# claserken/SISS

Hardware: AMD Instinct MI355X
Metric: unlearning samples/sec (= unlearning-steps/sec x batch x gpus), CelebA-HQ-256 DDPM SISS (higher is better)
Workload: dtype bf16; 1 GPU; delete_celeb.yaml: CelebA-HQ 256x256 DDPM UNet (113.7M params), SISS lambd=0.5, t=999, bf16, bs=16/GPU, GA=1, scaling_norm=500, AdamW lr 5e-6; loss_fn=importance_sampling_with_mixture, global_batch=16, grad_accum=1, parallelism=dp1, hipgraph=True

## Files before the change

### siss_amd/csrc/groupnorm.hip

```cpp
#include "nt_common.h"

namespace {

constexpr int kStatsDepth = 2;
constexpr int kThreads = 256;
constexpr int kMaxG = 32;
constexpr int kMaxC = 1024;

struct GNShape {
    int H, W, C, G, cpg, lpp, ppi;
    int chunk_px, nchunks;
    int ld, Gf, nslices;
    int ldx;
};

__device__ __forceinline__ long compact_row(int n, int pi, int H, int W) { return (long)n * H * W + pi; }

__device__ __forceinline__ void unpack8(u32x4_t r, float (&v)[8]) {
#pragma unroll
    for (int j = 0; j < 4; ++j) {
        v[2 * j] = __builtin_bit_cast(float, r[j] << 16);
        v[2 * j + 1] = __builtin_bit_cast(float, r[j] & 0xffff0000u);
    }
}
__device__ __forceinline__ u32x4_t pack8(const float (&v)[8]) {
    return u32x4_t{pack_bf2(v[0], v[1]), pack_bf2(v[2], v[3]), pack_bf2(v[4], v[5]), pack_bf2(v[6], v[7])};
}

struct PixelWalk {
    int pi, p1, x, W, ppi, dx, rw, drw;
    __device__ __forceinline__ PixelWalk(const GNShape& s, int chunk, int slot) {
        const int p0 = chunk * s.chunk_px;
        p1 = p0 + s.chunk_px; p1 = p1 < s.H * s.W ? p1 : s.H * s.W;
        pi = p0 + slot; W = s.W; ppi = s.ppi;
        const int y = pi / W; x = pi - y * W;
        const int dy = ppi / W; dx = ppi - dy * W;
        rw = (y + 1) * (W + 2) + (x + 1);
        drw = dy * (W + 2) + dx;
    }
    __device__ __forceinline__ bool ok() const { return pi < p1; }
    __device__ __forceinline__ int row() const { return rw; }
    __device__ __forceinline__ void next() {
        pi += ppi; x += dx; rw += drw;
        if (x >= W) { x -= W; rw += 2; }
    }
};

__device__ __forceinline__ unsigned boff(int row, unsigned row_bytes, unsigned lane_bytes) { return __umul24(row, row_bytes) + lane_bytes; }
__device__ __forceinline__ u32x4_t ld16(const bf16_t* base, unsigned off) {
    return *reinterpret_cast<const u32x4_t*>(reinterpret_cast<const char*>(base) + off);
}
__device__ __forceinline__ void st16(bf16_t* base, unsigned off, u32x4_t v) {
    *reinterpret_cast<u32x4_t*>(reinterpret_cast<char*>(base) + off) = v;
}

__device__ __forceinline__ void reduce_slots(const float (&v)[8], bool active, int slot, int cc, const GNShape& s,
                                             float* red, float* out) {
    if (active) {
        float* dst = red + slot * s.C + cc * 8;
        *reinterpret_cast<f32x4_t*>(dst) = f32x4_t{v[0], v[1], v[2], v[3]};
        *reinterpret_cast<f32x4_t*>(dst + 4) = f32x4_t{v[4], v[5], v[6], v[7]};
    }
    __syncthreads();
    for (int c = threadIdx.x; c < s.C; c += kThreads) {
        float a = 0.f;
        for (int sl = 0; sl < s.ppi; ++sl) a += red[sl * s.C + c];
        out[c] = a;
    }
    __syncthreads();
}

__global__ __launch_bounds__(kThreads) void gn_stats_kernel(const bf16_t* __restrict__ x, GNShape s,
                                                            float* __restrict__ partial) {
    __shared__ __attribute__((aligned(16))) float red[2048];
    __shared__ float ch_a[kMaxC], ch_b[kMaxC];
    const int n = blockIdx.y, chunk = blockIdx.x, tid = threadIdx.x;
    const int c0 = blockIdx.z * s.C;
    const int slot = tid / s.lpp, cc = tid - slot * s.lpp;
    const bool active = slot < s.ppi;
    float a[8] = {}, b[8] = {};
    if (active) {
        const bf16_t* base = x + (long)n * (s.H + 2) * (s.W + 2) * s.ldx + c0;
        const unsigned xb = s.ldx * 2, lb = cc * 16;
        PixelWalk w(s, chunk, slot);
        while (w.ok()) {
            const u32x4_t r0 = ld16(base, boff(w.row(), xb, lb));
            w.next();
// ... 106 lines not shown

__global__ __launch_bounds__(kThreads) void gn_qstats_finalize_kernel(
    const float* __restrict__ qsA, int qa, const float* __restrict__ qsB, int qb, int H, int W, int G, int cpg, float eps,
    float* __restrict__ mean, float* __restrict__ rstd) {
    const int n = blockIdx.x, tid = threadIdx.x, lane = tid & 63;
    const int g = blockIdx.y * 4 + (tid >> 6);
    if (g >= G) return;
    const long rpi = (long)(H + 2) * (W + 2);
    const int t0 = (int)(n * rpi / kQsTileRows), t1 = (int)(((n + 1) * rpi - 1) / kQsTileRows);
    const int qpg = cpg >> 2;
    const int items = (t1 - t0 + 1) * 2 * qpg;
    auto entry = [&](int it) -> float2 {
        if (it >= items) return float2{0.f, 0.f};
        const int hl = it / qpg, qi = it - hl * qpg;
        const int t = t0 + (hl >> 1), h = hl & 1;
        const int slot = (int)((long)t * kQsTileRows / rpi) == n ? 0 : 1;
        const int q = g * qpg + qi;
        const float* src = q < qa ? qsA : qsB;
        const int stride = q < qa ? qa : qb, qq = q < qa ? q : q - qa;
        return *reinterpret_cast<const float2*>(src + (((long)(2 * t + h) * 2 + slot) * stride + qq) * 2);
    };
    double a = 0.0, b = 0.0;
    for (int it = lane; it < items; it += 256) {
        const float2 e0 = entry(it), e1 = entry(it + 64), e2 = entry(it + 128), e3 = entry(it + 192);
        a += ((double)e0.x + (double)e1.x) + ((double)e2.x + (double)e3.x);
        b += ((double)e0.y + (double)e1.y) + ((double)e2.y + (double)e3.y);
    }
#pragma unroll
    for (int o = 32; o >= 1; o >>= 1) { a += __shfl_xor(a, o); b += __shfl_xor(b, o); }
    if (lane == 0) {
        const double cnt = (double)H * W * cpg;
        const double m = a / cnt;
        double var = b / cnt - m * m;
        var = var > 0 ? var : 0;
        mean[(long)n * G + g] = (float)m;
        rstd[(long)n * G + g] = (float)(1.0 / sqrt(var + (double)eps));
    }
}

__global__ __launch_bounds__(kThreads) void gn_quad_stats_kernel(const bf16_t* __restrict__ x, long ld, int M, int N, int rpi,
                                                                 float* __restrict__ qs) {
    __shared__ float red[8][kThreads];
    const int t = blockIdx.x >> 1, h = blockIdx.x & 1, tid = threadIdx.x;
    const int r0 = t * kQsTileRows + h * kQsHalfRows;
    int r1 = r0 + (h ? kQsTileRows - kQsHalfRows : kQsHalfRows);
    r1 = r1 < M ? r1 : M;
    const int bnd = (t * kQsTileRows / rpi + 1) * rpi;
    const int lpr = N >> 3, par = kThreads / lpr;
    const int rr = tid / lpr, cc = tid - rr * lpr;
    float a[8];
#pragma unroll
    for (int i = 0; i < 8; ++i) a[i] = 0.f;
    if (rr < par) {
        const bf16_t* src = x + cc * 8;
        for (int r = r0 + rr; r < r1; r += par) {
            const u32x4_t v4 = *reinterpret_cast<const u32x4_t*>(src + (long)r * ld);
            float v[8];
            unpack8(v4, v);
            const float w1 = r >= bnd ? 1.f : 0.f, w0 = 1.f - w1;
#pragma unroll
            for (int j = 0; j < 2; ++j) {
                const float s1 = (v[4 * j] + v[4 * j + 1]) + (v[4 * j + 2] + v[4 * j + 3]);
                const float s2 = (v[4 * j] * v[4 * j] + v[4 * j + 1] * v[4 * j + 1]) + (v[4 * j + 2] * v[4 * j + 2] + v[4 * j + 3] * v[4 * j + 3]);
                a[4 * j] += w0 * s1; a[4 * j + 1] += w0 * s2;
                a[4 * j + 2] += w1 * s1; a[4 * j + 3] += w1 * s2;
            }
        }
    }
#pragma unroll
    for (int i = 0; i < 8; ++i) red[i][tid] = a[i];
    __syncthreads();
    if (tid < lpr * 4) {
        const int c = tid >> 2, j = (tid >> 1) & 1, slot = tid & 1;
        float s1 = 0.f, s2 = 0.f;
        for (int k = 0; k < par; ++k) {
            s1 += red[4 * j + 2 * slot][k * lpr + c];
            s2 += red[4 * j + 2 * slot + 1][k * lpr + c];
        }
        const long e = ((long)(2 * t + h) * 2 + slot) * (N >> 2) + (2 * c + j);
        *reinterpret_cast<float2*>(qs + 2 * e) = float2{s1, s2};
    }
}

template <bool SILU, int SETS>
__global__ __launch_bounds__(kThreads) void gn_bwd_stats_kernel(
    const bf16_t* __restrict__ dy, const bf16_t* __restrict__ x, const float* __restrict__ gamma,
    const float* __restrict__ beta, const float* __restrict__ mean, const float* __restrict__ rstd,
    GNShape s, int nx, int dy_compact, int set_images, long set_stride, float* __restrict__ partial,
    float* __restrict__ dgamma, float* __restrict__ dbeta) {
    __shared__ __attribute__((aligned(16))) float red[2048];
    __shared__ float ch1[kMaxC], ch2[kMaxC];
    const int n = blockIdx.y, chunk = blockIdx.x, tid = threadIdx.x;
    const int c0 = blockIdx.z * s.C, g0 = blockIdx.z * s.G;
    const int slot = tid / s.lpp, cc = tid - slot * s.lpp;
    const bool active = slot < s.ppi;
    gamma += c0; beta += c0; dy += c0;
    float a1[SETS][8], a2[SETS][8];
#pragma unroll
    for (int k = 0; k < SETS; ++k)
#pragma unroll
        for (int e = 0; e < 8; ++e) { a1[k][e] = 0.f; a2[k][e] = 0.f; }
    if (active) {
        float mr[8], rs[8], ga[8], be[8], ga2[8], be2[8];
#pragma unroll
        for (int e = 0; e < 8; ++e) {
            const int c = cc * 8 + e, g = c / s.cpg;
            rs[e] = rstd[(long)n * s.Gf + g0 + g]; mr[e] = mean[(long)n * s.Gf + g0 + g] * rs[e];
            ga[e] = gamma[c]; be[e] = beta[c];
            ga2[e] = -1.44269504088896f * ga[e]; be2[e] = -1.44269504088896f * be[e];
        }
        const long rpi = (long)(s.H + 2) * (s.W + 2);
        const bf16_t* xbase = x + (long)n * rpi * s.ldx + c0;
        const bf16_t* dbase[SETS];
#pragma unroll
        for (int k = 0; k < SETS; ++k)
            dbase[k] = dy + (dy_compact ? (long)(k * nx + n) * s.H * s.W : (long)(k * nx + n) * rpi) * s.ld;
        const unsigned xb = s.ldx * 2, db = s.ld * 2, lb = cc * 16;
        PixelWalk w(s, chunk, slot);
        constexpr int DEPTH = kStatsDepth;
        u32x4_t bx[DEPTH], bd[DEPTH][SETS];
        bool have[DEPTH];
        auto issue = [&](const PixelWalk& q, u32x4_t& ox, u32x4_t (&od)[SETS]) {
            ox = ld16(xbase, boff(q.row(), xb, lb));
            const unsigned doff = boff(dy_compact ? q.pi : q.row(), db, lb);
#pragma unroll
            for (int k = 0; k < SETS; ++k) od[k] = ld16(dbase[k], doff);
        };
#pragma unroll
        for (int b2 = 0; b2 < DEPTH; ++b2) {
            bx[b2] = u32x4_t{0u, 0u, 0u, 0u};
#pragma unroll
            for (int k = 0; k < SETS; ++k) bd[b2][k] = u32x4_t{0u, 0u, 0u, 0u};
            have[b2] = w.ok();
            if (have[b2]) { issue(w, bx[b2], bd[b2]); w.next(); }
        }
        while (have[0]) {
#pragma unroll
            for (int b2 = 0; b2 < DEPTH; ++b2) {
                if (!have[b2]) break;
                const u32x4_t rx = bx[b2];
                u32x4_t rd[SETS];
#pragma unroll
                for (int k = 0; k < SETS; ++k) rd[k] = bd[b2][k];
                have[b2] = w.ok();
                if (have[b2]) { issue(w, bx[b2], bd[b2]); w.next(); }
                float v[8], q1[8], q2[8];
                unpack8(rx, v);
#pragma unroll
                for (int e = 0; e < 8; ++e) {
                    const float xh = v[e] * rs[e] - mr[e];
                    if (SILU) {
                        const float ex = __builtin_amdgcn_exp2f(xh * ga2[e] + be2[e]);
                        const float sg = __builtin_amdgcn_rcpf(1.f + ex);
                        const float z = xh * ga[e] + be[e];
                        q1[e] = sg * (1.f + z * (1.f - sg));
                    } else {
                        q1[e] = 1.f;
                    }
                    q2[e] = q1[e] * xh;
                }
#pragma unroll
                for (int k = 0; k < SETS; ++k) {
                    float d[8];
                    unpack8(rd[k], d);
#pragma unroll
                    for (int e = 0; e < 8; ++e) {
                        a1[k][e] += d[e] * q1[e]; a2[k][e] += d[e] * q2[e];
                    }
                }
            }
        }
    }
    for (int k = 0; k < SETS; ++k) {
        reduce_slots(a1[k], active, slot, cc, s, red, ch1);
        reduce_slots(a2[k], active, slot, cc, s, red, ch2);
        const int n2 = k * nx + n;
        if (tid < 2 * s.G) {
            const int g = tid >> 1;
            const float* src = (tid & 1) ? ch2 : ch1;
            float t = 0.f;
            for (int c = g * s.cpg; c < (g + 1) * s.cpg; ++c) t += src[c] * gamma[c];
            partial[(((long)n2 * s.nslices + blockIdx.z) * s.nchunks + chunk) * 2 * s.G + tid] = t;
        }
        const long so = (long)(n2 / set_images) * set_stride + c0;
        for (int i = tid; i < s.C; i += kThreads) {
            atomicAdd(dgamma + so + i, ch2[i]);
            atomicAdd(dbeta + so + i, ch1[i]);
        }
        __syncthreads();
    }
}

template <bool SILU>
__device__ __forceinline__ void gn_bwd_xhat(float v, float rs, float mr, float ga, float be, float& xh, float& dsl) {
#pragma clang fp contract(off)
    xh = fmaf(v, rs, -mr);
    dsl = (SILU ? dsilu_f(fmaf(xh, ga, be)) : 1.f) * ga;
}
__device__ __forceinline__ float gn_bwd_t(float d, float dsl, float xh, float rs, float m1, float m2) {
#pragma clang fp contract(off)
    return rs * fmaf(-xh, m2, fmaf(d, dsl, -m1));
}

template <bool SILU, int SETS, bool S2D>
__global__ __launch_bounds__(kThreads) void gn_bwd_apply_kernel(
    const bf16_t* __restrict__ dy, const bf16_t* __restrict__ x, const float* __restrict__ gamma,
    const float* __restrict__ beta, const float* __restrict__ mean, const float* __restrict__ rstd,
    const float* __restrict__ partial, GNShape s, int nx, int dy_compact, const bf16_t* __restrict__ accum,
    const bf16_t* __restrict__ accum2, bf16_t* __restrict__ dx, bf16_t* __restrict__ dx2, int split_c,
    int accumulate2, float* __restrict__ colsum, long colsum_ld, int pchunks) {
    __shared__ float sh_s1[SETS][kMaxG], sh_s2[SETS][kMaxG];
    __shared__ __attribute__((aligned(16))) float red[2048];
    __shared__ float chs[kMaxC];
    const int n = blockIdx.y, chunk = blockIdx.x, tid = threadIdx.x;
    const int c0 = blockIdx.z * s.C, g0 = blockIdx.z * s.G;
    gamma += c0; beta += c0;
    {
        __shared__ float fr[4][64];
        const double cnt = (double)s.H * s.W * s.cpg;
        for (int k = 0; k < SETS; ++k) {
            const int n2 = k * nx + n;
            fold_slab(partial + ((long)n2 * s.nslices + blockIdx.z) * pchunks * 2 * s.G, pchunks, s.G, fr);
            if (tid < s.G) {
                sh_s1[k][tid] = (float)(((double)fr[0][2 * tid] + fr[1][2 * tid] + fr[2][2 * tid] + fr[3][2 * tid]) / cnt);
                sh_s2[k][tid] = (float)(((double)fr[0][2 * tid + 1] + fr[1][2 * tid + 1] + fr[2][2 * tid + 1] + fr[3][2 * tid + 1]) / cnt);
            }
            __syncthreads();
        }
    }
    const int slot = tid / s.lpp, cc = tid - slot * s.lpp;
    const bool active = slot < s.ppi;
    float cs[SETS][8];
#pragma unroll
    for (int k = 0; k < SETS; ++k)
#pragma unroll
        for (int e = 0; e < 8; ++e) cs[k][e] = 0.f;
    if (active) {
        float mr[8], rs[8], ga[8], be[8], m1[SETS][8], m2[SETS][8];
#pragma unroll
        for (int e = 0; e < 8; ++e) {
            const int c = cc * 8 + e, g = c / s.cpg;
            rs[e] = rstd[(long)n * s.Gf + g0 + g]; mr[e] = mean[(long)n * s.Gf + g0 + g] * rs[e];
            ga[e] = gamma[c]; be[e] = beta[c];
#pragma unroll
            for (int k = 0; k < SETS; ++k) { m1[k][e] = sh_s1[k][g]; m2[k][e] = sh_s2[k][g]; }
        }
        const long rpi = (long)(s.H + 2) * (s.W + 2);
        const bf16_t* xbase = x + (long)n * rpi * s.ldx + c0;
        const int ch = c0 + cc * 8;
        const bool second = dx2 != nullptr && ch >= split_c;
        const int ostride = dx2 ? (second ? s.ld - split_c : split_c) : s.ld;
        const bool oacc = second && accumulate2;
        const bool any_oacc = dx2 != nullptr && accumulate2;
        const bf16_t* dbase[SETS]; const bf16_t* abase[SETS]; const bf16_t* bbase[SETS]; bf16_t* obase[SETS];
#pragma unroll
        for (int k = 0; k < SETS; ++k) {
            const long n2 = k * nx + n;
            dbase[k] = dy + c0 + (dy_compact ? n2 * s.H * s.W : n2 * rpi) * s.ld;
            abase[k] = accum ? accum + c0 + n2 * rpi * s.ld : nullptr;
            bbase[k] = accum2 ? accum2 + c0 + n2 * rpi * s.ld : nullptr;
            obase[k] = (second ? dx2 + (ch - split_c) : dx + ch) + n2 * rpi * ostride;
            if (S2D && !second) obase[k] = dx + ch + n2 * (long)((s.H >> 1) + 2) * ((s.W >> 1) + 2) * (4 * split_c);
        }
        const unsigned xb = s.ldx * 2, db = s.ld * 2, ob = ((S2D && !second) ? 4 * ostride : ostride) * 2, lb = cc * 16;
        const int wl2 = (s.W >> 1) + 2;
        const bool s2d_lane = S2D && !second;
        auto out_off = [&](int row, int yy, int xx) -> unsigned {
            if (!s2d_lane) return __umul24(row, ob);
            return __umul24(((yy >> 1) + 1) * wl2 + (xx >> 1) + 1, ob) + (unsigned)((((yy & 1) << 1) | (xx & 1)) * split_c * 2);
        };
        struct In { u32x4_t x, d[SETS], a[SETS], b[SETS], c[SETS]; };
        auto issue = [&](const PixelWalk& q, In& o) {
            o.x = ld16(xbase, boff(q.row(), xb, lb));
            const unsigned roff = boff(q.row(), db, lb);
            const unsigned doff = dy_compact ? boff(q.pi, db, lb) : roff;
            const unsigned ooff = __umul24(q.row(), ob);
#pragma unroll
            for (int k = 0; k < SETS; ++k) {
                o.d[k] = ld16(dbase[k], doff);
                if (accum) o.a[k] = ld16(abase[k], roff);
                if (accum2) o.b[k] = ld16(bbase[k], roff);
                if (any_oacc) o.c[k] = oacc ? ld16(obase[k], ooff) : u32x4_t{0u, 0u, 0u, 0u};
            }
        };
        PixelWalk w(s, chunk, slot);
        int yy = S2D ? w.pi / s.W : 0;
        const int dyi = S2D ? s.ppi / s.W : 0;
        In nxt;
        if (w.ok()) issue(w, nxt);
        while (w.ok()) {
            const In cur = nxt;
            const unsigned ooff = out_off(w.row(), yy, w.x);
            if (S2D) yy += dyi + (w.x + w.dx >= s.W ? 1 : 0);
            w.next();
            if (w.ok()) issue(w, nxt);
            float v[8], xh[8], dsl[8];
            unpack8(cur.x, v);
#pragma unroll
            for (int e = 0; e < 8; ++e) gn_bwd_xhat<SILU>(v[e], rs[e], mr[e], ga[e], be[e], xh[e], dsl[e]);
#pragma unroll
            for (int k = 0; k < SETS; ++k) {
                float d[8], o[8];
                unpack8(cur.d[k], d);
#pragma unroll
                for (int e = 0; e < 8; ++e) {
                    const float t = gn_bwd_t(d[e], dsl[e], xh[e], rs[e], m1[k][e], m2[k][e]);
                    cs[k][e] += t;
                    o[e] = t;
                }
                if (accum) {
                    float r[8];
                    unpack8(cur.a[k], r);
#pragma unroll
                    for (int e = 0; e < 8; ++e) o[e] += r[e];
                }
                if (accum2) {
                    float r[8];
                    unpack8(cur.b[k], r);
#pragma unroll
                    for (int e = 0; e < 8; ++e) o[e] += r[e];
                }
                if (any_oacc) {
                    float r[8];
                    unpack8(cur.c[k], r);
#pragma unroll
                    for (int e = 0; e < 8; ++e) o[e] += r[e];
                }
                st16(obase[k], ooff, pack8(o));
            }
        }
    }
    if (colsum) {
        for (int k = 0; k < SETS; ++k) {
            reduce_slots(cs[k], active, slot, cc, s, red, chs);
            for (int i = tid; i < s.C; i += kThreads) atomicAdd(colsum + (long)(k * nx + n) * colsum_ld + c0 + i, chs[i]);
            __syncthreads();
        }
    }
}

struct GNSCParams {
    const bf16_t* A; const bf16_t* Wt;
    const bf16_t* x; const bf16_t* dy; const bf16_t* accum2;
    const float* gamma; const float* beta; const f32x4_t* gconst;
    bf16_t* dx; bf16_t* dx2;
    long lda, ldx;
    int K, C, G, cpg, Mset, nx, sets, rpi, H, W, split_c, accumulate2;
    float inv_wp;
};
constexpr int kScTileBytes = 128 * kCRow;
constexpr int kScSmemBytes = kScTileBytes + 3 * kMaxG * 16;

__global__ __launch_bounds__(kThreads) void gn_bwd_sc_finalize_kernel(const float* __restrict__ partial, int pchunks,
                                                                      const float* __restrict__ mean, const float* __restrict__ rstd,
                                                                      int G, int nx, double cnt, f32x4_t* __restrict__ gconst) {
    __shared__ float fr[4][64];
    const int n2 = blockIdx.x, tid = threadIdx.x;
    fold_slab(partial + (long)n2 * pchunks * 2 * G, pchunks, G, fr);
    if (tid < G) {
        const int n = n2 % nx;
        const float s1 = (float)(((double)fr[0][2 * tid] + fr[1][2 * tid] + fr[2][2 * tid] + fr[3][2 * tid]) / cnt);
        const float s2 = (float)(((double)fr[0][2 * tid + 1] + fr[1][2 * tid + 1] + fr[2][2 * tid + 1] + fr[3][2 * tid + 1]) / cnt);
        const float r = rstd[(long)n * G + tid];
        gconst[(long)n2 * G + tid] = f32x4_t{r, mean[(long)n * G + tid] * r, s1, s2};
    }
}

template <bool SILU, bool S2D, bool EXTRA>
__global__ __launch_bounds__(kThreads, 3) void gn_bwd_sc_kernel(const GNSCParams p) {
    constexpr int BM = 128, kPieces = BM / 8 / 4;
    extern __shared__ __attribute__((aligned(16))) char smem[];
    const int tid = threadIdx.x, lane = tid & 63;
    const int w = __builtin_amdgcn_readfirstlane(tid >> 6);
    const int wm = w >> 1, wn = w & 1;
    const int tiles_n = (p.C + BN - 1) / BN, tiles_m = (p.Mset + BM - 1) / BM;
    const int nwg = tiles_n * tiles_m * p.sets;
    int bid = blockIdx.x;
    {
        const int q = nwg >> 3, r = nwg & 7, xcd = bid & 7, k = bid >> 3;
        bid = (xcd < r ? xcd * (q + 1) : r * (q + 1) + (xcd - r) * q) + k;
    }
    const int tn = bid % tiles_n, ts = bid / tiles_n;
    const int kset = ts % p.sets, tm = ts / p.sets;
    const int m0 = tm * BM, n0 = tn * BN;
    const long set_row0 = (long)kset * p.Mset;
    const bf16_t* A = p.A + set_row0 * p.lda;

    const bf16_t* asrc[kPieces];
    const bf16_t* wsrc[kPieces];
#pragma unroll
    for (int j = 0; j < kPieces; ++j) {
        const int row = (w * kPieces + j) * 8 + (lane >> 3);
        const int lc = (lane & 7) ^ ((row >> 1) & 7);
        int gr = m0 + row; gr = gr < p.Mset ? gr : p.Mset - 1;
        asrc[j] = A + (long)gr * p.lda + lc * 8;
        int gn = n0 + row; gn = gn < p.C ? gn : p.C - 1;
        wsrc[j] = p.Wt + (long)gn * p.K + lc * 8;
    }
    const int rpi = p.rpi;
    const int img0 = m0 / rpi;
    f32x4_t* cst = reinterpret_cast<f32x4_t*>(smem + kScTileBytes);
    if (tid < 3 * p.G) {
        const int slot = tid / p.G, g = tid - slot * p.G;
        int img = img0 + slot; img = img < p.nx ? img : p.nx - 1;
        cst[tid] = p.gconst[(long)(kset * p.nx + img) * p.G + g];
    }
    const int chunk = tid & 15, trow = tid >> 4;
    const int nc = n0 + chunk * 8;
    const bool cols = nc < p.C;
    float ga[8], be[8];
#pragma unroll
    for (int e = 0; e < 8; ++e) { ga[e] = cols ? p.gamma[nc + e] : 0.f; be[e] = cols ? p.beta[nc + e] : 0.f; }

    f32x4_t acc[4][4];
#pragma unroll
    for (int i = 0; i < 4; ++i)
#pragma unroll
        for (int j = 0; j < 4; ++j) acc[i][j] = f32x4_t{0.f, 0.f, 0.f, 0.f};
    const int frow = lane & 15, fq = lane >> 4;
    int a_off[4], w_off[4];
#pragma unroll
    for (int i = 0; i < 4; ++i) {
        const int ra = wm * 64 + i * 16 + frow;
        a_off[i] = ra * 128 + ((fq ^ ((ra >> 1) & 7)) << 4);
        const int rw = wn * 64 + i * 16 + frow;
        w_off[i] = BM * 128 + rw * 128 + ((fq ^ ((rw >> 1) & 7)) << 4);
    }
    const unsigned smem_a = lds_addr(smem);
    const int steps = p.K / BK;
    for (int s = 0; s < steps; ++s) {
        asm volatile("s_waitcnt lgkmcnt(0)" ::: "memory");
        __builtin_amdgcn_s_barrier();
#pragma unroll
        for (int j = 0; j < kPieces; ++j) glds16_asm(asrc[j] + s * BK, smem_a + (w * kPieces + j) * 1024);
#pragma unroll
        for (int j = 0; j < kPieces; ++j) glds16_asm(wsrc[j] + s * BK, smem_a + BM * 128 + (w * kPieces + j) * 1024);
        asm volatile("s_waitcnt vmcnt(0)" ::: "memory");
        __builtin_amdgcn_s_barrier();
#pragma unroll
// ... 43 lines not shown
    const int Wp = p.W + 2, Hp = p.H + 2;
    const int C = p.C;
    const bool second = p.dx2 != nullptr && nc >= p.split_c;
    const int ostride = p.dx2 ? (second ? C - p.split_c : p.split_c) : C;
    const bool oacc = EXTRA && second && p.accumulate2;
    const bool any_oacc = EXTRA && p.dx2 != nullptr && p.accumulate2;
    const bool s2d_lane = S2D && !second;
    bf16_t* const obase = second ? p.dx2 + (nc - p.split_c) : p.dx + nc;
    const int wl2 = (p.W >> 1) + 2;
    const long img2 = (long)((p.H >> 1) + 2) * wl2;
    const bf16_t* const xb = p.x + nc;
    const bf16_t* const db = p.dy + set_row0 * C + nc;
    const bf16_t* const bb = (EXTRA && p.accum2) ? p.accum2 + set_row0 * C + nc : nullptr;
    constexpr int kBatch = EXTRA ? 2 : 4;
    for (int it0 = 0; it0 < BM / 16; it0 += kBatch) {
        u32x4_t vx[kBatch], vd[kBatch], vb[EXTRA ? kBatch : 1], vc[EXTRA ? kBatch : 1];
        bf16_t* dst[kBatch];
        int state[kBatch];
        int slot_of[kBatch];
#pragma unroll
        for (int q = 0; q < kBatch; ++q) {
            const int row = (it0 + q) * 16 + trow;
            const int r = m0 + row;
            const int slot = (row >= b1) + (row >= b2);
            slot_of[q] = slot;
            const int img = img0 + slot;
            const int rem = r - img * rpi;
            const int y = (int)(((float)rem + 0.5f) * p.inv_wp), xq = rem - y * Wp;
            const bool halo = (y == 0) | (y == Hp - 1) | (xq == 0) | (xq == Wp - 1);
            state[q] = r >= p.Mset ? 0 : (halo ? (s2d_lane ? 0 : 1) : 2);
            vx[q] = vd[q] = u32x4_t{0u, 0u, 0u, 0u};
            if (EXTRA) vb[q] = vc[q] = u32x4_t{0u, 0u, 0u, 0u};
            if (s2d_lane) {
                const int yy = y - 1, xx = xq - 1;
                dst[q] = p.dx + nc + (((long)(kset * p.nx + img) * img2 + ((yy >> 1) + 1) * wl2 + (xx >> 1) + 1) * 4 + (((yy & 1) << 1) | (xx & 1))) * p.split_c;
            } else {
                dst[q] = obase + (set_row0 + r) * ostride;
            }
            if (state[q] == 2) {
                vx[q] = *reinterpret_cast<const u32x4_t*>(xb + (long)r * p.ldx);
                vd[q] = *reinterpret_cast<const u32x4_t*>(db + (long)r * C);
                if (EXTRA && bb) vb[q] = *reinterpret_cast<const u32x4_t*>(bb + (long)r * C);
                if (EXTRA && oacc) vc[q] = *reinterpret_cast<const u32x4_t*>(dst[q]);
            }
        }
#pragma unroll
        for (int q = 0; q < kBatch; ++q) {
            if (state[q] == 0) continue;
            u32x4_t out = u32x4_t{0u, 0u, 0u, 0u};
            if (state[q] == 2) {
                if (slot_of[q] != cur_slot) { cur_slot = slot_of[q]; load_consts(cur_slot); }
                const int row = (it0 + q) * 16 + trow;
                float v[8], d[8], pr[8], o[8];
                unpack8(vx[q], v);
                unpack8(vd[q], d);
                unpack8(*reinterpret_cast<const u32x4_t*>(smem + row * kCRow + chunk * 16), pr);
#pragma unroll
                for (int e = 0; e < 8; ++e) {
                    float xh, dsl;
                    gn_bwd_xhat<SILU>(v[e], rs[e], mr[e], ga[e], be[e], xh, dsl);
                    o[e] = gn_bwd_t(d[e], dsl, xh, rs[e], m1[e], m2[e]);
                }
#pragma unroll
                for (int e = 0; e < 8; ++e) o[e] += pr[e];
                if (EXTRA && bb) {
                    float r8[8];
                    unpack8(vb[q], r8);
#pragma unroll
                    for (int e = 0; e < 8; ++e) o[e] += r8[e];
                }
                if (EXTRA && any_oacc) {
                    float r8[8];
                    unpack8(vc[q], r8);
#pragma unroll
                    for (int e = 0; e < 8; ++e) o[e] += r8[e];
                }
                out = pack8(o);
            }
            *reinterpret_cast<u32x4_t*>(dst[q]) = out;
        }
    }
}

constexpr int kBlocksFwd = 768, kBlocksBwd = 512, kBlocksBwdStats = 767;

bool make_shape(int H, int W, int C, int G, GNShape& s, int N = 16, int blocks = kBlocksFwd) {
    if (H <= 0 || W <= 0 || C <= 0 || G <= 0 || G > kMaxG || C % G || C % 8) return false;
    s.H = H; s.W = W; s.ld = C; s.ldx = C; s.Gf = G; s.cpg = C / G;
    int gs = G;
    if (C > kMaxC) {
        int best = 0, best_util = -1;
        gs = 0;
        for (int d = G; d >= 1; --d) {
            if (G % d) continue;
            const int cs = d * s.cpg;
            if (cs > kMaxC || cs % 8) continue;
            const int lpp = cs / 8, util = (kThreads / lpp) * lpp;
            if (util * 10 >= kThreads * 9) { gs = d; break; }
            if (util > best_util) { best_util = util; best = d; }
        }
        if (gs == 0) gs = best;
        if (gs == 0) return false;
    }
    s.G = gs; s.C = gs * s.cpg; s.nslices = G / gs;
    s.lpp = s.C / 8;
    if (s.lpp > kThreads) return false;
    s.ppi = kThreads / s.lpp;
    const int px = H * W;
    int nch = (blocks + N * s.nslices - 1) / (N * s.nslices);
    const int max_by_work = (px + 16 * s.ppi - 1) / (16 * s.ppi);
    if (nch > max_by_work) nch = max_by_work;
    if (blocks == kBlocksBwd || blocks == kBlocksBwdStats) {
        const int by_work32 = (px + 32 * s.ppi - 1) / (32 * s.ppi);
        if (nch > by_work32 && (long)by_work32 * N * s.nslices >= 256) nch = by_work32;
    }
    if (nch > 256) nch = 256;
    if (nch < 1) nch = 1;
    s.chunk_px = (px + nch - 1) / nch;
    s.nchunks = (px + s.chunk_px - 1) / s.chunk_px;
    return true;
}

int g_use_slab = 1;

}

int siss_gn_slab_fwd(const void* x, const float* gamma, const float* beta, void* y, float* mean, float* rstd, int N, int H,
                     int W, int C, int G, float eps, int silu, int out_compact, int ldx, void* stream);
int siss_gn_slab_bwd(const void* dy, const void* x, const float* gamma, const float* beta, const float* mean,
                     const float* rstd, void* dx, const void* accum, const void* accum2, void* dx2, int split_c,
                     int accumulate2, float* dgamma, float* dbeta, float* colsum, long colsum_ld, int n2, int nx,
                     int set_images, long set_stride, int H, int W, int C, int G, int silu, int dy_compact, int ldx,
                     void* stream);
extern "C" {

int siss_groupnorm_set_slab(int on) {
    g_use_slab = on != 0;
    return g_use_slab;
}

long siss_gn_partial_words(int n, int H, int W, int C, int G) {
    GNShape s;
    if (!make_shape(H, W, C, G, s, 1)) return -1;
    return (long)n * s.nslices * s.nchunks * 2 * s.G;
}

int siss_quad_stats(const void* x, long ld, int M, int N, int rows_per_image, float* qs, void* stream) {
    SISS_CHECK_ARG(x && qs && M > 0 && N > 0 && N % 8 == 0 && N <= 8 * kThreads && ld >= N && ld % 8 == 0 && rows_per_image >= 256);
    SISS_CHECK_ARG((uintptr_t)x % 16 == 0 && (uintptr_t)qs % 8 == 0 && (N >> 3) * 4 <= kThreads);
    const int tiles = (M + kQsTileRows - 1) / kQsTileRows;
    gn_quad_stats_kernel<<<dim3(2 * tiles), kThreads, 0, (hipStream_t)stream>>>((const bf16_t*)x, ld, M, N, rows_per_image, qs);
    SISS_LAUNCH_RET();
}

int siss_groupnorm_fwd_qs(const void* x, const float* gamma, const float* beta, void* y, float* mean,
                          float* rstd, float* partial, const float* qsA, int ca, const float* qsB, int N, int H, int W,
                          int C, int G, float eps, int silu, int out_compact, int ldx, void* stream) {
    GNShape s;
    SISS_CHECK_ARG(!qsA || (ca > 0 && ca <= C && ca % 4 == 0 && (ca == C) == (qsB == nullptr)));
    SISS_CHECK_ARG(((uintptr_t)qsA | (uintptr_t)qsB) % 8 == 0);
    SISS_CHECK_ARG(x && gamma && beta && y && mean && rstd && partial && N > 0);
    SISS_CHECK_ARG(make_shape(H, W, C, G, s, N, kBlocksFwd));
    SISS_CHECK_ARG(ldx == 0 || (ldx >= C && ldx % 8 == 0));
    if (ldx) s.ldx = ldx;
    SISS_CHECK_ARG(((uintptr_t)x | (uintptr_t)y | (uintptr_t)partial) % 16 == 0);
    if (g_use_slab && s.nslices == 1) {
        const int rc = siss_gn_slab_fwd(x, gamma, beta, y, mean, rstd, N, H, W, C, G, eps, silu, out_compact, ldx, stream);
        if (rc >= 0) return rc;
    }
    hipStream_t st = (hipStream_t)stream;
    dim3 grid(s.nchunks, N, s.nslices);
    if (qsA && s.cpg % 4 == 0 && (long)(H + 2) * (W + 2) >= 256) {
        siss_count_dispatch(SISS_K_GN_QSTATS);
        gn_qstats_finalize_kernel<<<dim3(N, (G + 3) / 4), kThreads, 0, st>>>(qsA, ca / 4, qsB, (C - ca) / 4, H, W, G, s.cpg, eps,
                                                                             mean, rstd);
        partial = nullptr;
    } else
        gn_stats_kernel<<<grid, kThreads, 0, st>>>((const bf16_t*)x, s, partial);
    if (silu)
        gn_apply_kernel<true><<<grid, kThreads, 0, st>>>((const bf16_t*)x, gamma, beta, partial, s, eps, out_compact, (bf16_t*)y, mean, rstd);
    else
        gn_apply_kernel<false><<<grid, kThreads, 0, st>>>((const bf16_t*)x, gamma, beta, partial, s, eps, out_compact, (bf16_t*)y, mean, rstd);
    SISS_LAUNCH_RET();
}
int siss_groupnorm_fwd_ld(const void* x, const float* gamma, const float* beta, void* y, float* mean,
                          float* rstd, float* partial, int N, int H, int W, int C, int G, float eps,
                          int silu, int out_compact, int ldx, void* stream) {
    return siss_groupnorm_fwd_qs(x, gamma, beta, y, mean, rstd, partial, nullptr, C, nullptr, N, H, W, C, G, eps, silu,
                                 out_compact, ldx, stream);
}
int siss_groupnorm_fwd(const void* x, const float* gamma, const float* beta, void* y, float* mean,
                       float* rstd, float* partial, int N, int H, int W, int C, int G, float eps,
                       int silu, int out_compact, void* stream) {
    return siss_groupnorm_fwd_ld(x, gamma, beta, y, mean, rstd, partial, N, H, W, C, G, eps, silu, out_compact, 0, stream);
}

static int gn_bwd_launch(const void* dy, const void* x, const float* gamma, const float* beta,
                          const float* mean, const float* rstd, void* dx, const void* accum, const void* accum2,
                          void* dx2, int split_c, int accumulate2, float* dgamma,
                          float* dbeta, float* colsum, long colsum_ld, float* partial, int n2, int nx, int set_images,
                          long set_stride, int H, int W, int C, int G, int silu, int dy_compact, int ldx, int s2d, void* stream) {
    GNShape s;
    SISS_CHECK_ARG(!s2d || (dx2 && H % 2 == 0 && W % 2 == 0));
    SISS_CHECK_ARG(dy && x && gamma && beta && mean && rstd && dx && dgamma && dbeta && partial);
    SISS_CHECK_ARG(n2 > 0 && nx > 0 && set_images > 0 && n2 % set_images == 0);
    SISS_CHECK_ARG(n2 == nx || n2 == 2 * nx);
    SISS_CHECK_ARG(make_shape(H, W, C, G, s, nx, kBlocksBwd));
    SISS_CHECK_ARG(((uintptr_t)dy | (uintptr_t)x | (uintptr_t)dx | (uintptr_t)accum | (uintptr_t)accum2 | (uintptr_t)dx2) % 16 == 0);
    SISS_CHECK_ARG(!dx2 || (split_c > 0 && split_c < C && split_c % 8 == 0));
    SISS_CHECK_ARG(ldx == 0 || (ldx >= C && ldx % 8 == 0));
    SISS_CHECK_ARG((uintptr_t)partial % 16 == 0);
    if (ldx) s.ldx = ldx;
    if (!s2d && g_use_slab && s.nslices == 1 && (n2 == nx || n2 == 2 * nx) && n2 / set_images <= 2) {
        const int rc = siss_gn_slab_bwd(dy, x, gamma, beta, mean, rstd, dx, accum, accum2, dx2, split_c, accumulate2, dgamma, dbeta,
                                        colsum, colsum_ld, n2, nx, set_images, set_stride, H, W, C, G, silu, dy_compact, ldx, stream);
        if (rc >= 0) return rc;
    }
    hipStream_t st = (hipStream_t)stream;
    GNShape ss;
    SISS_CHECK_ARG(make_shape(H, W, C, G, ss, nx, kBlocksBwdStats));
    ss.ldx = s.ldx;
    dim3 grid(s.nchunks, nx, s.nslices), grid_s(ss.nchunks, nx, ss.nslices);
    const bf16_t* dyp = (const bf16_t*)dy; const bf16_t* xp = (const bf16_t*)x;
#define GN_BWD(SILU, SETS)                                                                                          \
    gn_bwd_stats_kernel<SILU, SETS><<<grid_s, kThreads, 0, st>>>(dyp, xp, gamma, beta, mean, rstd, ss, nx, dy_compact, \
                                                               set_images, set_stride, partial, dgamma, dbeta);    \
    if (s2d)                                                                                                        \
        gn_bwd_apply_kernel<SILU, SETS, true><<<grid, kThreads, 0, st>>>(dyp, xp, gamma, beta, mean, rstd, partial, s, nx,    \
                                                               dy_compact, (const bf16_t*)accum, (const bf16_t*)accum2, (bf16_t*)dx, (bf16_t*)dx2, split_c,  \
                                                               accumulate2, colsum, colsum_ld, ss.nchunks);                \
    else                                                                                                            \
        gn_bwd_apply_kernel<SILU, SETS, false><<<grid, kThreads, 0, st>>>(dyp, xp, gamma, beta, mean, rstd, partial, s, nx,    \
                                                               dy_compact, (const bf16_t*)accum, (const bf16_t*)accum2, (bf16_t*)dx, (bf16_t*)dx2, split_c,  \
                                                               accumulate2, colsum, colsum_ld, ss.nchunks)
    if (n2 == nx) { if (silu) { GN_BWD(true, 1); } else { GN_BWD(false, 1); } }
    else          { if (silu) { GN_BWD(true, 2); } else { GN_BWD(false, 2); } }
#undef GN_BWD
    SISS_LAUNCH_RET();
}
int siss_groupnorm_bwd_ld(const void* dy, const void* x, const float* gamma, const float* beta,
                          const float* mean, const float* rstd, void* dx, const void* accum, const void* accum2,
                          void* dx2, int split_c, int accumulate2, float* dgamma,
                          float* dbeta, float* colsum, long colsum_ld, float* partial, int n2, int nx, int set_images,
                          long set_stride, int H, int W, int C, int G, int silu, int dy_compact, int ldx, void* stream) {
    return gn_bwd_launch(dy, x, gamma, beta, mean, rstd, dx, accum, accum2, dx2, split_c, accumulate2, dgamma, dbeta, colsum, colsum_ld,
                         partial, n2, nx, set_images, set_stride, H, W, C, G, silu, dy_compact, ldx, 0, stream);
}
int siss_groupnorm_bwd_ld_s2d(const void* dy, const void* x, const float* gamma, const float* beta,
                              const float* mean, const float* rstd, void* dx, const void* accum, const void* accum2,
                              void* dx2, int split_c, int accumulate2, float* dgamma,
                              float* dbeta, float* colsum, long colsum_ld, float* partial, int n2, int nx, int set_images,
                              long set_stride, int H, int W, int C, int G, int silu, int dy_compact, int ldx, void* stream) {
    return gn_bwd_launch(dy, x, gamma, beta, mean, rstd, dx, accum, accum2, dx2, split_c, accumulate2, dgamma, dbeta, colsum, colsum_ld,
                         partial, n2, nx, set_images, set_stride, H, W, C, G, silu, dy_compact, ldx, 1, stream);
}
int siss_groupnorm_bwd(const void* dy, const void* x, const float* gamma, const float* beta,
                       const float* mean, const float* rstd, void* dx, const void* accum, const void* accum2,
                       void* dx2, int split_c, int accumulate2, float* dgamma,
                       float* dbeta, float* colsum, long colsum_ld, float* partial, int n2, int nx, int set_images,
                       long set_stride, int H, int W, int C, int G, int silu, int dy_compact, void* stream) {
    return siss_groupnorm_bwd_ld(dy, x, gamma, beta, mean, rstd, dx, accum, accum2, dx2, split_c, accumulate2, dgamma, dbeta,
                                 colsum, colsum_ld, partial, n2, nx, set_images, set_stride, H, W, C, G, silu, dy_compact, 0,
                                 stream);
}

int siss_groupnorm_bwd_sc(const void* dy, const void* x, const float* gamma, const float* beta, const float* mean,
                          const float* rstd, void* dx, const void* dout, long ldo, const void* wsc, int K, const void* accum2,
                          void* dx2, int split_c, int accumulate2, float* dgamma, float* dbeta, float* colsum, float* partial,
                          float* gconst, int n2, int nx, int set_images, long set_stride, int H, int W, int C, int G, int silu,
                          int s2d, int ldx, void* stream) {
    GNShape ss;
    SISS_CHECK_ARG(!colsum);
    SISS_CHECK_ARG(dy && x && gamma && beta && mean && rstd && dx && dout && wsc && dgamma && dbeta && partial && gconst);
    SISS_CHECK_ARG(!s2d || (dx2 && H % 2 == 0 && W % 2 == 0));
    SISS_CHECK_ARG(n2 > 0 && nx > 0 && set_images > 0 && n2 % set_images == 0 && (n2 == nx || n2 == 2 * nx));
    SISS_CHECK_ARG(K > 0 && K % BK == 0 && ldo >= K && ldo % 8 == 0);
    SISS_CHECK_ARG(make_shape(H, W, C, G, ss, nx, kBlocksBwdStats) && ss.nslices == 1);
    SISS_CHECK_ARG(((uintptr_t)dy | (uintptr_t)x | (uintptr_t)dx | (uintptr_t)dout | (uintptr_t)wsc | (uintptr_t)accum2 | (uintptr_t)dx2 |
                    (uintptr_t)partial | (uintptr_t)gconst) % 16 == 0);
    SISS_CHECK_ARG(!dx2 || (split_c > 0 && split_c < C && split_c % 8 == 0));
    SISS_CHECK_ARG(ldx == 0 || (ldx >= C && ldx % 8 == 0));
    const long rpi = (long)(H + 2) * (W + 2);
    SISS_CHECK_ARG(rpi >= 64 && nx * rpi < (1L << 31) - 256);
    if (ldx) ss.ldx = ldx;
    hipStream_t st = (hipStream_t)stream;
    static unsigned char attr_set[2][2][2][kMaxDevices];
    const bool extra = accum2 != nullptr || (dx2 && accumulate2);
    const bf16_t* dyp = (const bf16_t*)dy; const bf16_t* xp = (const bf16_t*)x;
    dim3 grid_s(ss.nchunks, nx, 1);
#define GN_SC_STATS(SILU, SETS) \
    gn_bwd_stats_kernel<SILU, SETS><<<grid_s, kThreads, 0, st>>>(dyp, xp, gamma, beta, mean, rstd, ss, nx, 0, set_images, set_stride, partial, dgamma, dbeta)
    if (n2 == nx) { if (silu) { GN_SC_STATS(true, 1); } else { GN_SC_STATS(false, 1); } }
    else          { if (silu) { GN_SC_STATS(true, 2); } else { GN_SC_STATS(false, 2); } }
#undef GN_SC_STATS
    gn_bwd_sc_finalize_kernel<<<n2, kThreads, 0, st>>>(partial, ss.nchunks, mean, rstd, G, nx, (double)H * W * ss.cpg, (f32x4_t*)gconst);
    GNSCParams p;
    p.A = (const bf16_t*)dout; p.Wt = (const bf16_t*)wsc; p.x = xp; p.dy = dyp; p.accum2 = (const bf16_t*)accum2;
    p.gamma = gamma; p.beta = beta; p.gconst = (const f32x4_t*)gconst; p.dx = (bf16_t*)dx; p.dx2 = (bf16_t*)dx2;
    p.lda = ldo; p.ldx = ss.ldx; p.K = K; p.C = C; p.G = G; p.cpg = ss.cpg; p.Mset = (int)(nx * rpi); p.nx = nx; p.sets = n2 / nx;
    p.rpi = (int)rpi; p.H = H; p.W = W; p.split_c = split_c; p.accumulate2 = accumulate2; p.inv_wp = 1.0f / (float)(W + 2);
    const unsigned blocks = (unsigned)(cdiv(p.Mset, 128) * cdiv(C, BN) * p.sets);
#define GN_SC_(SILU, S2D_, EX)                                                                                                \
    do {                                                                                                                      \
        if (siss_ensure_smem((const void*)gn_bwd_sc_kernel<SILU, S2D_, EX>, kScSmemBytes, attr_set[SILU][S2D_][EX]) != SISS_OK) return SISS_ERR_LAUNCH; \
        gn_bwd_sc_kernel<SILU, S2D_, EX><<<blocks, kThreads, kScSmemBytes, st>>>(p);                                           \
    } while (0)
#define GN_SC(SILU, S2D_) do { if (extra) GN_SC_(SILU, S2D_, true); else GN_SC_(SILU, S2D_, false); } while (0)
    if (silu) { if (s2d) GN_SC(true, true); else GN_SC(true, false); }
    else      { if (s2d) GN_SC(false, true); else GN_SC(false, false); }
#undef GN_SC
#undef GN_SC_
    siss_count_dispatch(SISS_K_GN_SC);
    SISS_LAUNCH_RET();
}

}
```

Before: 308.1 samples/sec.

## Replace GroupNorm backward per-block dgamma/dbeta atomics with partial buffer and fold

The backward stats kernel no longer issues per-channel atomicAdds into dgamma/dbeta from every chunk block. It writes per-chunk channel partials to a scratch buffer, and the apply or finalize kernel folds them column-wise with one atomic per channel. The change also stages per-group mean/rstd in registers when cpg is a multiple of 4, or in shared memory otherwise, instead of keeping eight per-element copies. It adds launch_bounds occupancy 4 and raises the stats block count. This cuts atomic contention and register pressure, at the cost of a larger partial workspace and extra fold work in downstream kernels.

```diff
diff --git a/siss_amd/csrc/groupnorm.hip b/siss_amd/csrc/groupnorm.hip
--- a/siss_amd/csrc/groupnorm.hip
+++ b/siss_amd/csrc/groupnorm.hip
@@ -3,6 +3,7 @@
 namespace {
 
 constexpr int kStatsDepth = 2;
+constexpr int kStatsDepthAnyCpg = 2;
 constexpr int kThreads = 256;
 constexpr int kMaxG = 32;
 constexpr int kMaxC = 1024;
@@ -275,12 +276,11 @@
     }
 }
 
-template <bool SILU, int SETS>
-__global__ __launch_bounds__(kThreads) void gn_bwd_stats_kernel(
+template <bool SILU, int SETS, bool Q4>
+__global__ __launch_bounds__(kThreads, 4) void gn_bwd_stats_kernel(
     const bf16_t* __restrict__ dy, const bf16_t* __restrict__ x, const float* __restrict__ gamma,
     const float* __restrict__ beta, const float* __restrict__ mean, const float* __restrict__ rstd,
-    GNShape s, int nx, int dy_compact, int set_images, long set_stride, float* __restrict__ partial,
-    float* __restrict__ dgamma, float* __restrict__ dbeta) {
+    GNShape s, int nx, int dy_compact, float* __restrict__ partial, float* __restrict__ chpart) {
     __shared__ __attribute__((aligned(16))) float red[2048];
     __shared__ float ch1[kMaxC], ch2[kMaxC];
     const int n = blockIdx.y, chunk = blockIdx.x, tid = threadIdx.x;
@@ -294,13 +294,27 @@
 #pragma unroll
         for (int e = 0; e < 8; ++e) { a1[k][e] = 0.f; a2[k][e] = 0.f; }
     if (active) {
-        float mr[8], rs[8], ga[8], be[8], ga2[8], be2[8];
+        float mr2[2] = {0.f, 0.f}, rs2[2] = {0.f, 0.f}, ga[8], be[8], ga2[8], be2[8];
+        const long go = (long)n * s.Gf + g0;
+#pragma unroll
+        for (int h = 0; Q4 && h < 2; ++h) {
+            const int g = (cc * 8 + 4 * h) / s.cpg;
+            rs2[h] = rstd[go + g]; mr2[h] = mean[go + g] * rs2[h];
+        }
 #pragma unroll
         for (int e = 0; e < 8; ++e) {
-            const int c = cc * 8 + e, g = c / s.cpg;
-            rs[e] = rstd[(long)n * s.Gf + g0 + g]; mr[e] = mean[(long)n * s.Gf + g0 + g] * rs[e];
+            const int c = cc * 8 + e;
             ga[e] = gamma[c]; be[e] = beta[c];
             ga2[e] = -1.44269504088896f * ga[e]; be2[e] = -1.44269504088896f * be[e];
+        }
+        if (!Q4) {
+#pragma unroll
+            for (int e = 0; e < 8; ++e) {
+                const int g = (cc * 8 + e) / s.cpg;
+                const float r = rstd[go + g];
+                red[e * kThreads + tid] = r;
+                (e < 4 ? ch1 : ch2)[(e & 3) * kThreads + tid] = mean[go + g] * r;
+            }
         }
         const long rpi = (long)(s.H + 2) * (s.W + 2);
         const bf16_t* xbase = x + (long)n * rpi * s.ldx + c0;
@@ -309,77 +323,112 @@
         for (int k = 0; k < SETS; ++k)
             dbase[k] = dy + (dy_compact ? (long)(k * nx + n) * s.H * s.W : (long)(k * nx + n) * rpi) * s.ld;
         const unsigned xb = s.ldx * 2, db = s.ld * 2, lb = cc * 16;
-        PixelWalk w(s, chunk, slot);
-        constexpr int DEPTH = kStatsDepth;
-        u32x4_t bx[DEPTH], bd[DEPTH][SETS];
-        bool have[DEPTH];
-        auto issue = [&](const PixelWalk& q, u32x4_t& ox, u32x4_t (&od)[SETS]) {
-            ox = ld16(xbase, boff(q.row(), xb, lb));
-            const unsigned doff = boff(dy_compact ? q.pi : q.row(), db, lb);
-#pragma unroll
-            for (int k = 0; k < SETS; ++k) od[k] = ld16(dbase[k], doff);
-        };
-#pragma unroll
-        for (int b2 = 0; b2 < DEPTH; ++b2) {
-            bx[b2] = u32x4_t{0u, 0u, 0u, 0u};
-#pragma unroll
-            for (int k = 0; k < SETS; ++k) bd[b2][k] = u32x4_t{0u, 0u, 0u, 0u};
-            have[b2] = w.ok();
-            if (have[b2]) { issue(w, bx[b2], bd[b2]); w.next(); }
-        }
-        while (have[0]) {
+        {
+            PixelWalk w(s, chunk, slot);
+            constexpr int DEPTH = Q4 ? kStatsDepth : kStatsDepthAnyCpg;
+            u32x4_t bx[DEPTH], bd[DEPTH][SETS];
+            bool have[DEPTH];
+            auto issue = [&](const PixelWalk& q, u32x4_t& ox, u32x4_t (&od)[SETS]) {
+                ox = ld16(xbase, boff(q.row(), xb, lb));
+                const unsigned doff = boff(dy_compact ? q.pi : q.row(), db, lb);
+#pragma unroll
+                for (int k = 0; k < SETS; ++k) od[k] = ld16(dbase[k], doff);
+            };
 #pragma unroll
             for (int b2 = 0; b2 < DEPTH; ++b2) {
-                if (!have[b2]) break;
-                const u32x4_t rx = bx[b2];
-                u32x4_t rd[SETS];
-#pragma unroll
-                for (int k = 0; k < SETS; ++k) rd[k] = bd[b2][k];
+                bx[b2] = u32x4_t{0u, 0u, 0u, 0u};
+#pragma unroll
+                for (int k = 0; k < SETS; ++k) bd[b2][k] = u32x4_t{0u, 0u, 0u, 0u};
                 have[b2] = w.ok();
                 if (have[b2]) { issue(w, bx[b2], bd[b2]); w.next(); }
-                float v[8], q1[8], q2[8];
-                unpack8(rx, v);
-#pragma unroll
-                for (int e = 0; e < 8; ++e) {
-                    const float xh = v[e] * rs[e] - mr[e];
-                    if (SILU) {
-                        const float ex = __builtin_amdgcn_exp2f(xh * ga2[e] + be2[e]);
-                        const float sg = __builtin_amdgcn_rcpf(1.f + ex);
-                        const float z = xh * ga[e] + be[e];
-                        q1[e] = sg * (1.f + z * (1.f - sg));
-                    } else {
-                        q1[e] = 1.f;
+            }
+            while (have[0]) {
+#pragma unroll
+                for (int b2 = 0; b2 < DEPTH; ++b2) {
+                    if (!have[b2]) break;
+                    const u32x4_t rx = bx[b2];
+                    u32x4_t rd[SETS];
+#pragma unroll
+                    for (int k = 0; k < SETS; ++k) rd[k] = bd[b2][k];
+                    have[b2] = w.ok();
+                    if (have[b2]) { issue(w, bx[b2], bd[b2]); w.next(); }
+                    float v[8], q1[8], q2[8];
+                    unpack8(rx, v);
+                    int po = tid;
+                    if (!Q4) asm volatile("" : "+v"(po));
+#pragma unroll
+                    for (int e = 0; e < 8; ++e) {
+                        float rse, mre;
+                        if constexpr (Q4) { rse = rs2[e >> 2]; mre = mr2[e >> 2]; }
+                        else { rse = red[e * kThreads + po]; mre = (e < 4 ? ch1 : ch2)[(e & 3) * kThreads + po]; }
+                        const float xh = v[e] * rse - mre;
+                        if (SILU) {
+                            const float ex = __builtin_amdgcn_exp2f(xh * ga2[e] + be2[e]);
+                            const float sg = __builtin_amdgcn_rcpf(1.f + ex);
+                            const float z = xh * ga[e] + be[e];
+                            q1[e] = sg * (1.f + z * (1.f - sg));
+                        } else {
+                            q1[e] = 1.f;
+                        }
+                        q2[e] = q1[e] * xh;
                     }
-                    q2[e] = q1[e] * xh;
-                }
-#pragma unroll
-                for (int k = 0; k < SETS; ++k) {
-                    float d[8];
-                    unpack8(rd[k], d);
-#pragma unroll
-                    for (int e = 0; e < 8; ++e) {
-                        a1[k][e] += d[e] * q1[e]; a2[k][e] += d[e] * q2[e];
+#pragma unroll
+                    for (int k = 0; k < SETS; ++k) {
+                        float d[8];
+                        unpack8(rd[k], d);
+#pragma unroll
+                        for (int e = 0; e < 8; ++e) {
+                            a1[k][e] += d[e] * q1[e]; a2[k][e] += d[e] * q2[e];
+                        }
                     }
                 }
             }
         }
     }
+    if (!Q4) __syncthreads();
+    int te = tid, lpp_e = s.lpp;
+    asm volatile("" : "+v"(te), "+s"(lpp_e));
+    const int slot_e = te / lpp_e, cc_e = te - slot_e * lpp_e;
+    const bool active_e = slot_e < s.ppi;
     for (int k = 0; k < SETS; ++k) {
-        reduce_slots(a1[k], active, slot, cc, s, red, ch1);
-        reduce_slots(a2[k], active, slot, cc, s, red, ch2);
+        reduce_slots(a1[k], active_e, slot_e, cc_e, s, red, ch1);
+        reduce_slots(a2[k], active_e, slot_e, cc_e, s, red, ch2);
         const int n2 = k * nx + n;
+        const long row = ((long)n2 * s.nslices + blockIdx.z) * s.nchunks + chunk;
         if (tid < 2 * s.G) {
             const int g = tid >> 1;
             const float* src = (tid & 1) ? ch2 : ch1;
             float t = 0.f;
             for (int c = g * s.cpg; c < (g + 1) * s.cpg; ++c) t += src[c] * gamma[c];
-            partial[(((long)n2 * s.nslices + blockIdx.z) * s.nchunks + chunk) * 2 * s.G + tid] = t;
-        }
-        const long so = (long)(n2 / set_images) * set_stride + c0;
-        for (int i = tid; i < s.C; i += kThreads) {
-            atomicAdd(dgamma + so + i, ch2[i]);
-            atomicAdd(dbeta + so + i, ch1[i]);
-        }
+            partial[row * 2 * s.G + tid] = t;
+        }
+        float* cp = chpart + row * 2 * s.C;
+        for (int i = tid; i < s.C; i += kThreads) { cp[i] = ch1[i]; cp[s.C + i] = ch2[i]; }
+        __syncthreads();
+    }
+}
+
+__device__ __forceinline__ void gn_fold_channel_partials(const float* __restrict__ chpart, int pchunks, int Cs, int nslices, int n2,
+                                                         int set_images, long set_stride, float* __restrict__ dgamma,
+                                                         float* __restrict__ dbeta, int bid, int nblocks, float* red) {
+    const int tid = threadIdx.x;
+    const int rows = set_images * pchunks, ncols = (n2 / set_images) * nslices * 2 * Cs;
+    for (int col = bid; col < ncols; col += nblocks) {
+        const int c = col % Cs;
+        int t = col / Cs;
+        const int which = t & 1; t >>= 1;
+        const int z = t % nslices, set = t / nslices;
+        const float* src = chpart + which * Cs + c;
+        float a = 0.f;
+#pragma unroll 4
+        for (int r = tid; r < rows; r += kThreads) {
+            const int i = r / pchunks, ck = r - i * pchunks;
+            a += src[((((long)set * set_images + i) * nslices + z) * pchunks + ck) * 2 * Cs];
+        }
+        a = wave_sum(a);
+        if ((tid & 63) == 0) red[tid >> 6] = a;
+        __syncthreads();
+        if (tid == 0) atomicAdd((which ? dgamma : dbeta) + set * set_stride + (long)z * Cs + c, (red[0] + red[1]) + (red[2] + red[3]));
         __syncthreads();
     }
 }
@@ -401,7 +450,8 @@
     const float* __restrict__ beta, const float* __restrict__ mean, const float* __restrict__ rstd,
     const float* __restrict__ partial, GNShape s, int nx, int dy_compact, const bf16_t* __restrict__ accum,
     const bf16_t* __restrict__ accum2, bf16_t* __restrict__ dx, bf16_t* __restrict__ dx2, int split_c,
-    int accumulate2, float* __restrict__ colsum, long colsum_ld, int pchunks) {
+    int accumulate2, float* __restrict__ colsum, long colsum_ld, int pchunks, const float* __restrict__ chpart, int set_images,
+    long set_stride, float* __restrict__ dgamma, float* __restrict__ dbeta) {
     __shared__ float sh_s1[SETS][kMaxG], sh_s2[SETS][kMaxG];
     __shared__ __attribute__((aligned(16))) float red[2048];
     __shared__ float chs[kMaxC];
@@ -410,6 +460,8 @@
     gamma += c0; beta += c0;
     {
         __shared__ float fr[4][64];
+        gn_fold_channel_partials(chpart, pchunks, s.C, s.nslices, SETS * nx, set_images, set_stride, dgamma, dbeta,
+                                 (blockIdx.z * gridDim.y + blockIdx.y) * gridDim.x + blockIdx.x, gridDim.x * gridDim.y * gridDim.z, fr[0]);
         const double cnt = (double)s.H * s.W * s.cpg;
         for (int k = 0; k < SETS; ++k) {
             const int n2 = k * nx + n;
@@ -546,8 +598,15 @@
 
 __global__ __launch_bounds__(kThreads) void gn_bwd_sc_finalize_kernel(const float* __restrict__ partial, int pchunks,
                                                                       const float* __restrict__ mean, const float* __restrict__ rstd,
-                                                                      int G, int nx, double cnt, f32x4_t* __restrict__ gconst) {
+                                                                      int G, int nx, double cnt, f32x4_t* __restrict__ gconst,
+                                                                      const float* __restrict__ chpart, int C, int n2tot, int set_images,
+                                                                      long set_stride, float* __restrict__ dgamma, float* __restrict__ dbeta) {
     __shared__ float fr[4][64];
+    if ((int)blockIdx.x >= n2tot) {
+        gn_fold_channel_partials(chpart, pchunks, C, 1, n2tot, set_images, set_stride, dgamma, dbeta, blockIdx.x - n2tot,
+                                 gridDim.x - n2tot, fr[0]);
+        return;
+    }
     const int n2 = blockIdx.x, tid = threadIdx.x;
     fold_slab(partial + (long)n2 * pchunks * 2 * G, pchunks, G, fr);
     if (tid < G) {
@@ -757,7 +816,7 @@
     }
 }
 
-constexpr int kBlocksFwd = 768, kBlocksBwd = 512, kBlocksBwdStats = 767;
+constexpr int kBlocksFwd = 768, kBlocksBwd = 512, kBlocksBwdStats = 1023;
 
 bool make_shape(int H, int W, int C, int G, GNShape& s, int N = 16, int blocks = kBlocksFwd) {
     if (H <= 0 || W <= 0 || C <= 0 || G <= 0 || G > kMaxG || C % G || C % 8) return false;
@@ -817,7 +876,9 @@
 long siss_gn_partial_words(int n, int H, int W, int C, int G) {
     GNShape s;
     if (!make_shape(H, W, C, G, s, 1)) return -1;
-    return (long)n * s.nslices * s.nchunks * 2 * s.G;
+    int cap = (H * W + 16 * s.ppi - 1) / (16 * s.ppi);
+    cap = cap > 256 ? 256 : (cap < 1 ? 1 : cap);
+    return (long)n * s.nslices * cap * 2 * (s.G + s.C);
 }
 
 int siss_quad_stats(const void* x, long ld, int M, int N, int rows_per_image, float* qs, void* stream) {
@@ -895,21 +956,24 @@
     GNShape ss;
     SISS_CHECK_ARG(make_shape(H, W, C, G, ss, nx, kBlocksBwdStats));
     ss.ldx = s.ldx;
+    float* const chpart = partial + (long)n2 * ss.nslices * ss.nchunks * 2 * ss.G;
     dim3 grid(s.nchunks, nx, s.nslices), grid_s(ss.nchunks, nx, ss.nslices);
     const bf16_t* dyp = (const bf16_t*)dy; const bf16_t* xp = (const bf16_t*)x;
-#define GN_BWD(SILU, SETS)                                                                                          \
-    gn_bwd_stats_kernel<SILU, SETS><<<grid_s, kThreads, 0, st>>>(dyp, xp, gamma, beta, mean, rstd, ss, nx, dy_compact, \
-                                                               set_images, set_stride, partial, dgamma, dbeta);    \
+#define GN_BWD(SILU, SETS, Q4_)                                                                                      \
+    gn_bwd_stats_kernel<SILU, SETS, Q4_><<<grid_s, kThreads, 0, st>>>(dyp, xp, gamma, beta, mean, rstd, ss, nx, dy_compact, \
+                                                               partial, chpart);                                    \
     if (s2d)                                                                                                        \
         gn_bwd_apply_kernel<SILU, SETS, true><<<grid, kThreads, 0, st>>>(dyp, xp, gamma, beta, mean, rstd, partial, s, nx,    \
                                                                dy_compact, (const bf16_t*)accum, (const bf16_t*)accum2, (bf16_t*)dx, (bf16_t*)dx2, split_c,  \
-                                                               accumulate2, colsum, colsum_ld, ss.nchunks);                \
+                                                               accumulate2, colsum, colsum_ld, ss.nchunks, chpart, set_images, set_stride, dgamma, dbeta); \
     else                                                                                                            \
         gn_bwd_apply_kernel<SILU, SETS, false><<<grid, kThreads, 0, st>>>(dyp, xp, gamma, beta, mean, rstd, partial, s, nx,    \
                                                                dy_compact, (const bf16_t*)accum, (const bf16_t*)accum2, (bf16_t*)dx, (bf16_t*)dx2, split_c,  \
-                                                               accumulate2, colsum, colsum_ld, ss.nchunks)
-    if (n2 == nx) { if (silu) { GN_BWD(true, 1); } else { GN_BWD(false, 1); } }
-    else          { if (silu) { GN_BWD(true, 2); } else { GN_BWD(false, 2); } }
+                                                               accumulate2, colsum, colsum_ld, ss.nchunks, chpart, set_images, set_stride, dgamma, dbeta)
+#define GN_BWD_(SILU, SETS) do { if (ss.cpg % 4 == 0) { GN_BWD(SILU, SETS, true); } else { GN_BWD(SILU, SETS, false); } } while (0)
+    if (n2 == nx) { if (silu) GN_BWD_(true, 1); else GN_BWD_(false, 1); }
+    else          { if (silu) GN_BWD_(true, 2); else GN_BWD_(false, 2); }
+#undef GN_BWD_
 #undef GN_BWD
     SISS_LAUNCH_RET();
 }
@@ -963,12 +1027,17 @@
     const bool extra = accum2 != nullptr || (dx2 && accumulate2);
     const bf16_t* dyp = (const bf16_t*)dy; const bf16_t* xp = (const bf16_t*)x;
     dim3 grid_s(ss.nchunks, nx, 1);
-#define GN_SC_STATS(SILU, SETS) \
-    gn_bwd_stats_kernel<SILU, SETS><<<grid_s, kThreads, 0, st>>>(dyp, xp, gamma, beta, mean, rstd, ss, nx, 0, set_images, set_stride, partial, dgamma, dbeta)
-    if (n2 == nx) { if (silu) { GN_SC_STATS(true, 1); } else { GN_SC_STATS(false, 1); } }
-    else          { if (silu) { GN_SC_STATS(true, 2); } else { GN_SC_STATS(false, 2); } }
+    float* const chpart = partial + (long)n2 * ss.nchunks * 2 * G;
+    const int ncols = (n2 / set_images) * 2 * C, fold_blocks = ncols < 512 ? ncols : 512;
+#define GN_SC_STATS_(SILU, SETS, Q4_) \
+    gn_bwd_stats_kernel<SILU, SETS, Q4_><<<grid_s, kThreads, 0, st>>>(dyp, xp, gamma, beta, mean, rstd, ss, nx, 0, partial, chpart)
+#define GN_SC_STATS(SILU, SETS) do { if (ss.cpg % 4 == 0) GN_SC_STATS_(SILU, SETS, true); else GN_SC_STATS_(SILU, SETS, false); } while (0)
+    if (n2 == nx) { if (silu) GN_SC_STATS(true, 1); else GN_SC_STATS(false, 1); }
+    else          { if (silu) GN_SC_STATS(true, 2); else GN_SC_STATS(false, 2); }
 #undef GN_SC_STATS
-    gn_bwd_sc_finalize_kernel<<<n2, kThreads, 0, st>>>(partial, ss.nchunks, mean, rstd, G, nx, (double)H * W * ss.cpg, (f32x4_t*)gconst);
+#undef GN_SC_STATS_
+    gn_bwd_sc_finalize_kernel<<<n2 + fold_blocks, kThreads, 0, st>>>(partial, ss.nchunks, mean, rstd, G, nx, (double)H * W * ss.cpg,
+                                                                     (f32x4_t*)gconst, chpart, C, n2, set_images, set_stride, dgamma, dbeta);
     GNSCParams p;
     p.A = (const bf16_t*)dout; p.Wt = (const bf16_t*)wsc; p.x = xp; p.dy = dyp; p.accum2 = (const bf16_t*)accum2;
     p.gamma = gamma; p.beta = beta; p.gconst = (const f32x4_t*)gconst; p.dx = (bf16_t*)dx; p.dx2 = (bf16_t*)dx2;
```

New measurement: 309.1 samples/sec (median of 5 runs). About the same (+0.3%).
